# cocowy1/Cost-Volume-Aggregation-in-Stereo-Matching-Revisited

Measured on AMD Instinct MI355X. Metric: cost-volumes/sec (fwd+bwd) at 544x960 D=192, higher is better.
Workload: dtype f32

## Files before the change

### cost-volume-aggregation-in-stereo-matching-revisited_amd/csrc/abi.hip

```cpp
#include "dca_common.h"

extern "C" int dca_abi_version(void) { return DCA_ABI_VERSION; }

extern "C" int dca_tile_walk(long tiles, int grid, int wg, int* walk) {
  DCA_REQUIRE(walk && tiles >= 0 && tiles < DCA_TILES_END && grid > 0 && wg >= 0 && wg < grid);
  const DcaTileWalk w = dca_tile_walk_of(tiles, (unsigned)grid, (unsigned)wg);
  walk[0] = w.begin; walk[1] = w.end; walk[2] = w.step;
  return 0;
}
```

### cost-volume-aggregation-in-stereo-matching-revisited_amd/csrc/conv3d_wgrad_s2_f16x2.hip

```cpp
#include "dca_frag.h"
#include "dca_tiles.h"
#include <type_traits>

namespace {

constexpr int NT = 2;
constexpr int TH = 4, TW = 16;
constexpr int NROW = TH;
constexpr int FD = 3, FH = 2 * TH + 1, NFROW = FD * FH;
constexpr int FV = 2 * TW + 1;
constexpr int VB = 64;
constexpr int X_TERM = NFROW * FV * VB;
constexpr int Y_BLK = NROW * TW * VB;
constexpr int Y_TERM = 2 * Y_BLK;
constexpr int X_OFF = 0, Y_OFF = NT * X_TERM;
constexpr int LDS_BYTES = Y_OFF + NT * Y_TERM;
constexpr int NXQ = NFROW * 8 * 4;
constexpr int KXQ = (NXQ + 511) / 512;
constexpr int NXE = NFROW * 4;
constexpr int NYQ = 2 * NROW * 4 * 4;
static_assert(NXQ - 512 + NYQ <= 512, "coarse items fit behind the second round of fine items");

struct WS2Args {
  const float* x;
  const float* dy;
  float* part;
  int N, Cx, Cy, D, H, W;
  int Do, Ho, Wo;
  int nTD, nTH, nTW, nCxT, nCyP;
  const int* xexps;
  const int* yexps;
};

__global__ __launch_bounds__(512) void wgrad3s2_f16x2_kernel(WS2Args a) {
  extern __shared__ __attribute__((aligned(16))) char smem[];
  const int tid = threadIdx.x, lane = tid & 63, wv = tid >> 6, l31 = lane & 31, half = lane >> 5;
  const int blk = wv >> 2, wq = wv & 3;
  const int ct = blockIdx.y, cyp = ct / a.nCxT, cx0 = (ct % a.nCxT) * 32, cy0 = cyp * 64;
  const bool blk_on = cy0 + 32 * blk < a.Cy;

  const DcaTileWalk walk = dca_my_tile_walk((long)a.N * a.nTD * a.nTH * a.nTW);
  const int t_begin = walk.begin, t_end = walk.end, t_step = walk.step;

  f32x16 acc[7];
#pragma unroll
  for (int j = 0; j < 7; ++j)
#pragma unroll
    for (int r = 0; r < 16; ++r) acc[j][r] = 0.f;

  const int cstride = a.D * a.H * a.W, ystride = a.Do * a.Ho * a.Wo;
  const long xsample = (long)a.Cx * cstride, ysample = (long)a.Cy * ystride;

  const int q4 = (lane & 15) >> 2, chb = (16 * ((lane >> 4) & 1) + 4 * (lane & 3)) * 2;
  const int lane_off_x = (2 * (8 * half + q4)) * VB + chb;
  const int lane_off_y = (8 * half + q4) * VB + chb;

  float4 rq[KXQ][8];
  float re[8];
  int* ex_lds = (int*)(smem + LDS_BYTES);
  if (tid < 32) ex_lds[tid] = (cx0 + tid < a.Cx) ? dca_coherent_loadi(a.xexps + cx0 + tid) : 0;
  else if (tid < 96) ex_lds[tid] = (cy0 + tid - 32 < a.Cy) ? dca_coherent_loadi(a.yexps + cy0 + tid - 32) : 0;
  __syncthreads();
  const int yu = tid - (NXQ - 512);
  auto decode = [&](int tile, int& n, int& d0, int& h0, int& w0) __attribute__((always_inline)) {
    dca_tile_decode<1, TH, TW>(tile, a.nTD, a.nTH, a.nTW, n, d0, h0, w0);
  };
  auto load_tile = [&](int n, int d0, int h0, int w0, int part = -1) __attribute__((always_inline)) {
    const __amdgpu_buffer_rsrc_t xr = dca_rsrc(a.x + (long)n * xsample, xsample * 4);
    const __amdgpu_buffer_rsrc_t yr = dca_rsrc(a.dy + (long)n * ysample, ysample * 4);
#pragma unroll
    for (int k = 0; k < KXQ; ++k) {
      if ((part == 0 && k >= 1) || (part == 1 && k < 1)) continue;
      const int it = tid + 512 * k, cg = it & 3, quad = (it >> 2) & 7, frow = it >> 5;
      const int d = 2 * d0 - 1 + frow / FH, h = 2 * h0 - 1 + frow % FH, w = 2 * w0 + 4 * quad, c0 = cx0 + cg * 8;
      const int ok = (int)(it < NXQ) & (int)((unsigned)d < (unsigned)a.D) & (int)((unsigned)h < (unsigned)a.H) & (int)(w + 3 < a.W);
      const int off = (c0 * cstride + (d * a.H + h) * a.W + w) * 4;
      if (512 * k + (tid & ~63) < NXQ) {
#pragma unroll
        for (int j = 0; j < 8; ++j) rq[k][j] = dca_bload4(xr, off + j * cstride * 4, ok & (int)(c0 + j < a.Cx));
      }
    }
    if (part == 0) return;
    if ((tid & ~63) < NXE + 63) {
      const int cg = tid & 3, frow = tid >> 2, c0 = cx0 + cg * 8;
      const int d = 2 * d0 - 1 + frow / FH, h = 2 * h0 - 1 + frow % FH, w = 2 * w0 - 1;
      const int ok = (int)(tid < NXE) & (int)((unsigned)d < (unsigned)a.D) & (int)((unsigned)h < (unsigned)a.H) &
                     (int)((unsigned)w < (unsigned)a.W);
      const int off = (c0 * cstride + (d * a.H + h) * a.W + w) * 4;
#pragma unroll
      for (int j = 0; j < 8; ++j) re[j] = dca_bload1(xr, off + j * cstride * 4, ok & (int)(c0 + j < a.Cx));
    }
    if ((unsigned)yu < (unsigned)NYQ) {
      const int cg = yu & 3, quad = (yu >> 2) & 3, row = (yu >> 4) & 3, by = yu >> 6;
      const int h = h0 + row, w = w0 + 4 * quad, c0 = cy0 + 32 * by + cg * 8;
      const int ok = (int)(h < a.Ho) & (int)(w + 3 < a.Wo);
      const int off = (c0 * ystride + (d0 * a.Ho + h) * a.Wo + w) * 4;
#pragma unroll
      for (int j = 0; j < 8; ++j) rq[1][j] = dca_bload4(yr, off + j * ystride * 4, ok & (int)(c0 + j < a.Cy));
    }
  };
  auto split_word = [&](const float (&v)[8], const int* exp8, char* dst, int term_stride) __attribute__((always_inline)) {
    const int4 e0 = *(const int4*)exp8, e1 = *(const int4*)(exp8 + 4);
    const int ex[8] = {e0.x, e0.y, e0.z, e0.w, e1.x, e1.y, e1.z, e1.w};
    f16x8 hv, lv;
#pragma unroll
    for (int j = 0; j < 8; ++j) {
      _Float16 h, l;
      x2_split(v[j], ex[j], h, l);
      hv[j] = h; lv[j] = l;
    }
    *(f16x8*)dst = hv;
    *(f16x8*)(dst + term_stride) = lv;
  };
  auto quad_words = [&](const float4 (&q)[8], const int* ex, char* dst, int term_stride) __attribute__((always_inline)) {
    const float* q0 = (const float*)&q[0];
#pragma unroll
    for (int vv = 0; vv < 4; ++vv) {
      const float v[8] = {q0[vv], q0[4 + vv], q0[8 + vv], q0[12 + vv], q0[16 + vv], q0[20 + vv], q0[24 + vv], q0[28 + vv]};
      split_word(v, ex, dst + vv * VB, term_stride);
    }
  };
  auto store_tile = [&]() __attribute__((always_inline)) {
#pragma unroll
    for (int k = 0; k < KXQ; ++k) {
      const int it = tid + 512 * k, cg = it & 3, quad = (it >> 2) & 7, frow = it >> 5;
      if (it < NXQ) quad_words(rq[k], ex_lds + cg * 8, smem + X_OFF + (frow * FV + 1 + 4 * quad) * VB + cg * 16, X_TERM);
    }
    if (tid < NXE) {
      const int cg = tid & 3, frow = tid >> 2;
      const float v[8] = {re[0], re[1], re[2], re[3], re[4], re[5], re[6], re[7]};
      split_word(v, ex_lds + cg * 8, smem + X_OFF + (frow * FV) * VB + cg * 16, X_TERM);
    }
    if ((unsigned)yu < (unsigned)NYQ) {
      const int cg = yu & 3, quad = (yu >> 2) & 3, row = (yu >> 4) & 3, by = yu >> 6;
      quad_words(rq[1], ex_lds + 32 + 32 * by + cg * 8, smem + Y_OFF + by * Y_BLK + (row * TW + 4 * quad) * VB + cg * 16, Y_TERM);
    }
  };

  auto mfma_tile = [&](auto WQC, bool more, int next_tile) __attribute__((always_inline)) {
    constexpr int WQ = decltype(WQC)::value;
    constexpr int TAP0 = 7 * WQ, TAP1 = (TAP0 + 7 < 27) ? TAP0 + 7 : 27, NTAP = TAP1 - TAP0;
#pragma unroll 1
    for (int i = 0; i < NROW; ++i) {
      if ((i == 1 || i == 2) && more) {
        int nn, nd0, nh0, nw0;
        decode(next_tile, nn, nd0, nh0, nw0);
        load_tile(nn, nd0, nh0, nw0, i - 1);
      }
      if (blk_on) {
        const char* yb = smem + Y_OFF + blk * Y_BLK + (i * TW) * VB + lane_off_y;
        const char* xb = smem + X_OFF + ((2 * i) * FV) * VB + lane_off_x;
        f16x8 ay[NT];
#pragma unroll
        for (int term = 0; term < NT; ++term) ay[term] = tr_frag(yb + term * Y_TERM, 4 * VB);
        f16x8 bx[2][NT];
        auto load_b = [&](int tap, int slot) __attribute__((always_inline)) {
          const int kd = tap / 9, kh = (tap / 3) % 3, kw = tap % 3;
#pragma unroll
          for (int term = 0; term < NT; ++term)
            bx[slot][term] = tr_frag(xb + term * X_TERM + ((kd * FH + kh) * FV + kw) * VB, 8 * VB);
        };
        load_b(TAP0, 0);
#pragma unroll
        for (int j = 0; j < NTAP; ++j) {
          const int cur = j & 1;
          if (j + 1 < NTAP) load_b(TAP0 + j + 1, cur ^ 1);
          acc[j] = __builtin_amdgcn_mfma_f32_32x32x16_f16(ay[0], bx[cur][1], acc[j], 0, 0, 0);
          acc[j] = __builtin_amdgcn_mfma_f32_32x32x16_f16(ay[1], bx[cur][0], acc[j], 0, 0, 0);
          acc[j] = __builtin_amdgcn_mfma_f32_32x32x16_f16(ay[0], bx[cur][0], acc[j], 0, 0, 0);
          if (j + 1 < NTAP) {
            __builtin_amdgcn_sched_group_barrier(0x100, 2, 0);
            __builtin_amdgcn_sched_group_barrier(0x008, 1, 0);
            __builtin_amdgcn_sched_group_barrier(0x100, 2, 0);
            __builtin_amdgcn_sched_group_barrier(0x008, 2, 0);
          }
          __builtin_amdgcn_sched_barrier(0);
        }
      }
    }
  };

  if (t_begin < t_end) {
    int n, d0, h0, w0;
    decode(t_begin, n, d0, h0, w0);
    load_tile(n, d0, h0, w0);
    store_tile();
    __syncthreads();
#pragma unroll 1
    for (int tile = t_begin; tile < t_end; tile += t_step) {
      const bool more = tile + t_step < t_end;
      switch (wq) {
        case 0: mfma_tile(std::integral_constant<int, 0>{}, more, tile + t_step); break;
        case 1: mfma_tile(std::integral_constant<int, 1>{}, more, tile + t_step); break;
        case 2: mfma_tile(std::integral_constant<int, 2>{}, more, tile + t_step); break;
        default: mfma_tile(std::integral_constant<int, 3>{}, more, tile + t_step); break;
      }
      __syncthreads();
      if (more) store_tile();
      __syncthreads();
    }
  }

  if (blk_on) {
    const int xe_l = ex_lds[l31];
    int ninv[16];
#pragma unroll
    for (int r = 0; r < 16; ++r) ninv[r] = -(ex_lds[32 + 32 * blk + (r & 3) + 8 * (r >> 2) + 4 * half] + xe_l);
    const int nCT32 = a.nCxT * ((a.Cy + 31) / 32), ct32 = (2 * cyp + blk) * a.nCxT + (ct % a.nCxT);
    float* slab = a.part + ((long)blockIdx.x * nCT32 + ct32) * 27 * 1024;
#pragma unroll
    for (int j = 0; j < 7; ++j) {
      const int tap = 7 * wq + j;
      if (tap < 27) {
#pragma unroll
        for (int r = 0; r < 16; ++r) {
          const int co = (r & 3) + 8 * (r >> 2) + 4 * half;
          slab[tap * 1024 + co * 32 + l31] = ldexpf(acc[j][r], ninv[r]);
        }
      }
    }
  }
}

struct WS2Geom {
  int Do, Ho, Wo, nCxT, nCyP, nWG, nCT, nblk;
  DcaTileGrid t;
  long part_floats;
};
WS2Geom ws2_geometry(int N, int Cx, int Cy, int D, int H, int W) {
  WS2Geom g;
  g.Do = (D + 1) / 2; g.Ho = (H + 1) / 2; g.Wo = (W + 1) / 2;
  g.t = dca_tile_grid<1, TH, TW>(N, g.Do, g.Ho, g.Wo);
  g.nCxT = cdiv(Cx, 32); g.nCyP = cdiv(Cy, 64);
  g.nWG = g.nCxT * g.nCyP;
  g.nCT = g.nCxT * cdiv(Cy, 32);
  g.nblk = dca_persistent_grid(g.t.tiles, g.nWG);
  g.part_floats = (long)g.nblk * g.nCT * 27 * 1024;
  return g;
}

}

extern "C" long dca_conv3d_wgrad_s2_x2_workspace(int N, int Cx, int Cy, int D, int H, int W) {
  if (N <= 0 || Cx <= 0 || Cy <= 0 || D <= 0 || H <= 0 || W <= 0) return 0;
  return ws2_geometry(N, Cx, Cy, D, H, W).part_floats;
}

extern "C" int dca_conv3d_wgrad_s2_x2(const float* f, const int* f_exps, const float* c, const int* c_exps,
                                      float* part, float* dw, int N, int Cx, int Cy, int D, int H, int W, long s_cy,
                                      long s_cx, hipStream_t stream) {
  DCA_REQUIRE(f && c && part && dw && f_exps && c_exps && N > 0 && Cx > 0 && Cy > 0 && D > 0 && H > 0 && W > 0);
  WS2Args a;
  a.x = f; a.dy = c; a.part = part; a.xexps = f_exps; a.yexps = c_exps;
  a.N = N; a.Cx = Cx; a.Cy = Cy; a.D = D; a.H = H; a.W = W;
  const WS2Geom g = ws2_geometry(N, Cx, Cy, D, H, W);
  a.Do = g.Do; a.Ho = g.Ho; a.Wo = g.Wo;
  DCA_REQUIRE(W % 4 == 0 && a.Wo % 4 == 0 && ((((uintptr_t)f | (uintptr_t)c) & 15) == 0));
  DCA_REQUIRE((long)Cx * D * H * W * 4 < 0x7ffffff0L && (long)Cy * a.Do * a.Ho * a.Wo * 4 < 0x7ffffff0L);
  a.nTD = g.t.nTD; a.nTH = g.t.nTH; a.nTW = g.t.nTW; a.nCxT = g.nCxT; a.nCyP = g.nCyP;
  DCA_REQUIRE(g.t.fits() && g.nWG <= 65535);
  const int lds = LDS_BYTES + 96 * 4;
  hipError_t e = hipFuncSetAttribute((const void*)wgrad3s2_f16x2_kernel, hipFuncAttributeMaxDynamicSharedMemorySize, lds);
  if (e != hipSuccess) return (int)e;
  hipLaunchKernelGGL(wgrad3s2_f16x2_kernel, dim3(g.nblk, g.nWG), dim3(512), lds, stream, a);
  int st = dca_launch_status();
  if (st) return st;
  return dca_internal_wgrad_reduce(part, dw, g.nblk, g.nCxT, g.nCT, 27, Cy, Cx, s_cy, s_cx, stream);
}
```

### cost-volume-aggregation-in-stereo-matching-revisited_amd/csrc/dca_tiles.h

```cpp
#pragma once
#include <hip/hip_runtime.h>

struct DcaTileWalk {
  int begin, end, step;
};

__host__ __device__ __forceinline__ DcaTileWalk dca_tile_walk_of(long T, unsigned grid, unsigned wg) {
  const int nx = grid >= 8 ? 8 : 1, xcd = wg % nx;
  const int cnt = (grid - xcd + nx - 1) / nx;
  DcaTileWalk w;
  w.begin = (int)(T * xcd / nx) + wg / nx; w.end = (int)(T * (xcd + 1) / nx); w.step = cnt;
  return w;
}
__device__ __forceinline__ DcaTileWalk dca_my_tile_walk(long T) { return dca_tile_walk_of(T, gridDim.x, blockIdx.x); }

template <int TD, int TH, int TW>
__host__ __device__ __forceinline__ void dca_tile_decode(int tile, int nTD, int nTH, int nTW, int& n, int& d0, int& h0, int& w0) {
  const int tw = tile % nTW; tile /= nTW;
  const int th = tile % nTH; tile /= nTH;
  const int td = tile % nTD;
  n = tile / nTD;
  d0 = td * TD; h0 = th * TH; w0 = tw * TW;
}

struct DcaTileStep {
  int tile, chunk, n, d0, h0, w0;
};
template <int TD, int TH, int TW>
__host__ __device__ __forceinline__ void dca_tile_advance(DcaTileStep& c, int nchunk, const DcaTileWalk& walk, int nTD, int nTH,
                                                          int nTW) {
  if (c.chunk + 1 < nchunk) { ++c.chunk; return; }
  c.chunk = 0;
  c.tile += walk.step;
  if (c.tile < walk.end) dca_tile_decode<TD, TH, TW>(c.tile, nTD, nTH, nTW, c.n, c.d0, c.h0, c.w0);
}

constexpr long DCA_TILES_END = 0x7fffffffL;
struct DcaTileGrid {
  int nTD, nTH, nTW;
  long tiles;
  bool fits() const { return tiles < DCA_TILES_END; }
};
template <int TD, int TH, int TW>
static inline DcaTileGrid dca_tile_grid(int N, int D, int H, int W) {
  DcaTileGrid t;
  t.nTD = (D + TD - 1) / TD; t.nTH = (H + TH - 1) / TH; t.nTW = (W + TW - 1) / TW;
  t.tiles = (long)N * t.nTD * t.nTH * t.nTW;
  return t;
}
```

### include/dca_hip.h

```cpp
#ifndef DCA_HIP_H
#define DCA_HIP_H

#include <hip/hip_runtime_api.h>

#ifdef __cplusplus
extern "C" {
#endif

#define DCA_ABI_VERSION 21
int dca_abi_version(void);

#define DCA_BF16 1
#define DCA_FP16 2

int dca_gwc_volume_fwd(const float* ref, const float* tgt, float* vol, int B, int C, int H, int W, int maxdisp,
                       int num_groups, hipStream_t stream);
int dca_gwc_volume_bwd(const float* gvol, const float* ref, const float* tgt, float* gref, float* gtgt, int B, int C,
                       int H, int W, int maxdisp, int num_groups, hipStream_t stream);
long dca_gwc_volume_bwd_rows(int B, int C, int H, int W, int maxdisp, int num_groups);
int dca_concat_volume_fwd(const float* ref, const float* tgt, float* vol, int B, int C, int H, int W, int maxdisp,
                          hipStream_t stream);
int dca_concat_volume_bwd(const float* gvol, float* gref, float* gtgt, int B, int C, int H, int W, int maxdisp,
                          hipStream_t stream);

int dca_cost_volume_fwd(const float* const* refs, const float* const* tgts, const int* seg_channels, int nseg,
                        const float* cref, const float* ctgt, int Cc, void* vol, int B, int H, int W, int maxdisp,
                        int num_groups, int dtype, unsigned* vmax, hipStream_t stream);

int dca_softargmin_fwd(const float* x, float* out, int B, int K, long HW, int mode, hipStream_t stream);
int dca_softargmin_bwd(const float* aux, const float* g, float* gx, int B, int K, long HW, int mode,
                       hipStream_t stream);

int dca_up_softargmin_fwd(const float* logits, float* disp, int B, int n, int hc, int wc, int scale, hipStream_t stream);
int dca_up_softargmin_bwd(const float* logits, const float* gdisp, float* g1, float* glogits, int B, int n, int hc,
                          int wc, int scale, hipStream_t stream);

int dca_conv3d_prep_weight(const float* w, float* wt, int A, int B, int Apad, int Bpad, int K, int src_ab, int flip,
                           int Btotal, int b_off, hipStream_t stream);
int dca_conv3d_forward(const float* x, const float* x2, const float* wt, float* y, const float* scale,
                       const float* shift, const float* res_pre, const float* res_post, float slope, int N, int Cin,
                       int C1, int Cout, int CinPad, int CoutTotal, int co_off, int Di, int Hi, int Wi, int Do, int Ho,
                       int Wo, int ksize, int stride, int transposed, hipStream_t stream);
long dca_conv3d_wgrad_workspace(int N, int Cx, int Cy, int Do, int Ho, int Wo, int ksize, int stride);
int dca_conv3d_wgrad(const float* x, const float* dy, float* part, float* dw, int N, int Cx, int Cy, int Di, int Hi,
                     int Wi, int Do, int Ho, int Wo, int ksize, int stride, long s_cy, long s_cx, hipStream_t stream);

long dca_conv1_bwd_fused_workspace(int N, long S, int two);
int dca_conv1_bwd_fused(const float* dz, const float* y, const float* stats, const float* dgb, float slope, int training,
                        const float* x, const float* x2, const float* w, float* part, float* dx, float* dx2, float* dw,
                        long s_cy, long s_cx, int N, int C1, int C2, int Cout, long S, hipStream_t stream);

long dca_conv1_x3_weight_bytes(int A);
int dca_conv1_x3_prep_weight(const float* w, void* wfrag, int A, int Bn, int src_ab, int Btotal, int b_off,
                             hipStream_t stream);
int dca_conv1_x3_forward(const float* x, const float* x2, const void* wfrag, float* y, const float* scale,
                         const float* shift, const float* res_pre, const float* res_post, float slope, int N, int C1,
                         int C2, int Cout, int CoutTotal, int co_off, long S, hipStream_t stream);

int dca_conv3d_prep_many(const void* table, int n, hipStream_t stream);

int dca_tile_walk(long tiles, int grid, int wg, int* walk);

long dca_conv3d_x3_weight_bytes(int Cin, int Cout);
int dca_conv3d_x3_prep_weight(const float* w, void* wx, int A, int B, int src_ab, int flip, hipStream_t stream);
int dca_conv3d_x3_forward(const float* x, const void* wx, float* y, const float* scale, const float* shift,
                          const float* res_pre, const float* res_post, float slope, int N, int Cin, int Cout, int D,
                          int H, int W, hipStream_t stream);

int dca_deconv3d_x3_forward(const float* x, const void* wx, float* y, const float* scale, const float* shift,
                            const float* res_pre, const float* res_post, float slope, int N, int Cin, int Cout, int Di,
                            int Hi, int Wi, hipStream_t stream);

long dca_conv3d_x3_stats_chunks(int N, int Cout, int D, int H, int W);
int dca_conv3d_x3_forward_stats(const float* x, const void* wx, float* y, double* stat_part, int N, int Cin, int Cout,
                                int D, int H, int W, hipStream_t stream);
long dca_conv1_x3_stats_chunks(int N, long S);
int dca_conv1_x3_forward_stats(const float* x, const float* x2, const void* wfrag, float* y, double* stat_part, int N,
                               int C1, int C2, int Cout, int CoutTotal, int co_off, long S, hipStream_t stream);
long dca_deconv3d_x3_stats_chunks(int N, int Di, int Hi, int Wi);
int dca_deconv3d_x3_forward_stats(const float* x, const void* wx, float* y, double* stat_part, int N, int Cin, int Cout,
                                  int Di, int Hi, int Wi, hipStream_t stream);
int dca_bn_finalize_centered(const double* part, int nchunk, const float* gamma, const float* beta, float* running_mean,
                             float* running_var, float momentum, float eps, float* stats, int* zexps,
                             const unsigned* rpre_slots, int rpre_n, const unsigned* rpost_slots, int rpost_n, int C,
                             hipStream_t stream);

long dca_conv3d_wgrad_x3_workspace(int N, int Cx, int Cy, int D, int H, int W);
int dca_conv3d_wgrad_x3(const float* x, const float* dy, float* part, float* dw, int N, int Cx, int Cy, int D, int H,
                        int W, long s_cy, long s_cx, hipStream_t stream);

#define DCA_AMAX_CSLOTS 1024
int dca_cmax_f32(const float* x, int N, int C, long S, unsigned* slots, hipStream_t stream);
int dca_cmax_exps(const unsigned* slots, int nslots, int C, int* exps, hipStream_t stream);
long dca_conv3d_x2_weight_bytes(int Cin, int Cout);
int dca_conv3d_x2_prep_weight(const float* w, void* wx, int A, int B, int src_ab, int flip, const unsigned* x_slots,
                              int nslots, int* xexps, hipStream_t stream);
int dca_conv3d_x2_forward(const void* x, int packed, const int* xexps, const void* wx, float* y, const float* scale,
                          const float* shift, const float* res_pre, const float* res_post, float slope, unsigned* y_cmax,
                          int N, int Cin, int Cout, int D, int H, int W, hipStream_t stream);
long dca_conv3d_x2_stats_chunks(int N, int Cout, int D, int H, int W);
int dca_conv3d_x2_forward_stats(const void* x, int packed, const int* xexps, const void* wx, float* y, double* stat_part,
                                int N, int Cin, int Cout, int D, int H, int W, hipStream_t stream);
long dca_conv3d_wgrad_s2_x2_workspace(int N, int Cx, int Cy, int D, int H, int W);
int dca_conv3d_wgrad_s2_x2(const float* f, const int* f_exps, const float* c, const int* c_exps, float* part,
                           float* dw, int N, int Cx, int Cy, int D, int H, int W, long s_cy, long s_cx, hipStream_t stream);
long dca_conv3d_s2x2_weight_bytes(int Cin, int Cout);
int dca_conv3d_s2x2_prep_weight(const float* w, void* wx, int A, int B, int src_ab, int flip, const unsigned* x_slots,
                                int nslots, int* xexps, hipStream_t stream);
long dca_conv3d_s2x2_out_slots(int N, int Cout, int Di, int Hi, int Wi);
int dca_conv3d_s2x2_forward(const float* x, const int* xexps, const void* wx, float* y, const float* scale, const float* shift,
                            float slope, const float* res_post, unsigned* y_cmax, int N, int Cin, int Cout, int Di, int Hi, int Wi,
                            hipStream_t stream);
long dca_conv3d_wgrad_x2_workspace(int N, int Cx, int Cy, int D, int H, int W);
int dca_conv3d_wgrad_x2(const void* x, int x_packed, const int* xexps, const void* dy, int dy_packed, const int* yexps,
                        float* part, float* dw, int N, int Cx, int Cy, int D, int H, int W, long s_cy, long s_cx,
                        hipStream_t stream);

int dca_conv3d_c1_gather(const float* T, float* y, int N, int D, int H, int W, hipStream_t stream);
int dca_conv3d_c1_wgrad(const float* x, const float* dy, float* part, float* dw, int N, int C, int D, int H, int W,
                        hipStream_t stream);
int dca_conv3d_c1_expand(const float* dy, float* G, int N, int D, int H, int W, hipStream_t stream);
int dca_conv3d_c1_bwd_data(const float* dy, const float* w, float* dx, int N, int C, int D, int H, int W,
                           hipStream_t stream);

int dca_bn_num_chunks(int C, long S);
int dca_bn_pack_chunks(int C, long S);
int dca_bn_stats(const float* x, double* part, int N, int C, long S, hipStream_t stream);
int dca_bn_finalize(const double* part, int nchunk, double count, const float* gamma, const float* beta,
                    float* running_mean, float* running_var, float momentum, float eps, int training, float* stats,
                    int* zexps, const unsigned* rpre_slots, int rpre_n, const unsigned* rpost_slots, int rpost_n, int C,
                    hipStream_t stream);
int dca_bn_apply(const float* y, const float* stats, const float* res_pre, const float* res_post, float* z, int N,
                 int C, long S, float slope, unsigned* zmax, unsigned* ymax, hipStream_t stream);
int dca_bn_apply_pack(const float* y, const float* stats, const int* zexps, void* zp, int N, int C, long S, float slope,
                      unsigned* ymax, const float* res_pre, const float* res_post, float* zf, unsigned* zmax,
                      hipStream_t stream);
int dca_bn_backward(const float* dz, const float* y, const float* res_pre, const float* stats, double* part,
                    float* dgb, float* dy, float* g_out, int N, int C, long S, float slope, int training,
                    unsigned* dmax, hipStream_t stream);
int dca_bn_backward_reduce(const float* dz, const float* y, const float* stats, double* part, float* dgb, int N, int C,
                           long S, float slope, int training, hipStream_t stream);
int dca_bn_backward_pack(const float* dz, const float* y, const float* stats, double* part, float* dgb, void* dyp,
                         int* dyexps, unsigned* gmax, const unsigned* ymax, int ymax_slots, int N, int C, long S,
                         float slope, int training, hipStream_t stream);
int dca_bn_skip_max(const float* y_r, const float* stats_r, int N, int C, long S, unsigned* slots, hipStream_t stream);
int dca_bn_apply_pack_skip(const float* y, const float* stats, const int* zexps, void* zp, int N, int C, long S, float slope,
                           unsigned* ymax, const float* y_r, const float* stats_r, const float* res_post, float* zf,
                           unsigned* zmax, hipStream_t stream);
int dca_bn_backward_skip(const float* dz, const float* y, const float* y_r, const float* stats, const float* stats_r,
                         double* part, double* part_r, float* dgb, float* dgb_r, float* dy, float* g_out, int N, int C,
                         long S, float slope, int training, unsigned* dmax, hipStream_t stream);

int dca_avgpool3d_fwd(const float* x, float* y, long NC, int Di, int Hi, int Wi, hipStream_t stream);
int dca_avgpool3d_bwd(const float* gy, float* gx, const float* res, const float* res2, long NC, int Di, int Hi, int Wi,
                     hipStream_t stream);

int dca_trilinear_fwd(const float* x, float* y, long NC, int Di, int Hi, int Wi, int scale, hipStream_t stream);
int dca_trilinear_bwd(const float* gy, float* gx, long NC, int Di, int Hi, int Wi, int scale, hipStream_t stream);

int dca_context_inject_fwd(const float* x, const float* preds, float* key, int* kstar, float* e, float* pm,
                           float* denom, float* part, int B, int C, int n, long HW, hipStream_t stream);
int dca_context_inject_bwd(const float* dkey, const float* x, const float* preds, const int* kstar, const float* e,
                           const float* pm, const float* denom, float* dx, float* dpreds, float* dw, float* T,
                           float* part, int B, int C, int n, long HW, hipStream_t stream);

int dca_disp_attention_fwd(const float* q, const float* k, const float* v, float* out, int B, int C, int n, long HW,
                           hipStream_t stream);
int dca_disp_attention_bwd(const float* q, const float* k, const float* v, const float* dout, float* dq, float* dk,
                           float* dv, int B, int C, int n, long HW, hipStream_t stream);

int dca_convex_up4_fwd(const float* mask_logits, const float* disp, float* up, int B, int h, int w, hipStream_t stream);
int dca_convex_up4_bwd(const float* mask_logits, const float* disp, const float* gup, float* glogits, float* gdisp,
                       float* wk, int B, int h, int w, hipStream_t stream);

long dca_focal_loss_workspace(int nlev, int B, long HW);
int dca_focal_loss_fwd(const float* const* ests, const float* weights, int nlev, const float* gt, double* work,
                       float* out, int B, int K, long HW, float focal_coefficient, hipStream_t stream);
int dca_focal_loss_bwd(const float* const* ests, float* const* gests, const float* weights, int nlev, const float* gt,
                       const double* work, const float* gloss, int B, int K, long HW, float focal_coefficient,
                       hipStream_t stream);

long dca_conv3d_lp_weight_bytes(int Cin, int Cout);
int dca_conv3d_lp_prep_weight(const float* w, void* wx, int A, int B, int src_ab, int flip, int dtype,
                              hipStream_t stream);
int dca_conv3d_lp_forward(const void* x, const void* wx, void* y, const float* scale, const float* shift,
                          const void* res_pre, const void* res_post, float slope, int N, int Cin, int Cout, int D, int H,
                          int W, int dtype, int in_f32, int out_f32, hipStream_t stream);

long dca_conv1_lp_weight_bytes(int C1, int C2);
int dca_conv1_lp_prep_weight(const float* w, void* wfrag, int Cout, int C1, int C2, int dtype, hipStream_t stream);
int dca_conv1_lp_forward(const void* x, const void* x2, const void* wfrag, void* y, const float* scale,
                         const float* shift, const void* res_pre, const void* res_post, float slope, int N, int C1,
                         int C2, int Cout, long S, int dtype, int out_f32, hipStream_t stream);

int dca_conv3d_forward_mixed(const void* x, const float* wt, void* y, const float* scale, const float* shift,
                             const void* res_pre, const void* res_post, float slope, int N, int Cin, int Cout, int CinPad,
                             int Di, int Hi, int Wi, int Do, int Ho, int Wo, int transposed, int dtype,
                             hipStream_t stream);
long dca_conv3d_s2_lp_weight_bytes(int Cin);
int dca_conv3d_s2_lp_prep_weight(const float* w, void* wx, int Cin, int Cout, int dtype, hipStream_t stream);
int dca_conv3d_s2_lp_forward(const void* x, const void* wx, float* y, const float* scale, const float* shift, float slope,
                             int N, int Cin, int Cout, int D, int H, int W, int dtype, hipStream_t stream);
int dca_deconv3d_lp_forward(const float* x, const void* wx, void* y, const float* scale, const float* shift,
                            const void* res_pre, const void* res_post, float slope, int N, int Cin, int Cout, int Di,
                            int Hi, int Wi, int dtype, hipStream_t stream);
int dca_avgpool3d_lp_fwd(const void* x, float* y, long NC, int Di, int Hi, int Wi, int dtype, hipStream_t stream);
int dca_trilinear_up2_lp_fwd(const float* x, void* y, long NC, int Di, int Hi, int Wi, int dtype, hipStream_t stream);

#define DCA_EVAL_REC 8
long dca_disp_metrics_workspace(int B, int H, int W);
int dca_disp_metrics(const float* pred, const float* gt, const unsigned char* mask, double* rec, void* workspace, int B,
                     int H, int W, int top_pad, int right_pad, float maxdisp, hipStream_t stream);
#define DCA_EVAL_MAX_CLASSES 64
int dca_region_confusion(const float* vol0, const float* vol1, const float* vol2, const float* gt, long long* cm,
                         int nvol, int B, int C, int hp, int wp, int H, int W, hipStream_t stream);
#define DCA_EVAL_BATCHES 0
#define DCA_EVAL_SUMS 1
#define DCA_EVAL_IMG_KEPT 11
#define DCA_EVAL_IMG_EPE 12
#define DCA_EVAL_IMG_D1 13
#define DCA_EVAL_IMG_THRES 14
#define DCA_EVAL_IMG_SEEN 17
#define DCA_EVAL_PIXELS 18
#define DCA_EVAL_STATE_HEAD 32
long dca_eval_state_len(int C);
int dca_eval_accumulate(const double* rec, const long long* cm, double* state, int B, int nvol, int C, int H, int W,
                        hipStream_t stream);

int dca_frame_hist(const unsigned char* left, const unsigned char* right, unsigned* hist, int H, int W, int C,
                   hipStream_t stream);
int dca_frame_lut(const unsigned* hist, long n_pixels, float* lut, double* stats, hipStream_t stream);
int dca_frame_apply(const unsigned char* left, const unsigned char* right, const float* lut, float* out_left,
                    float* out_right, int H, int W, int C, int Hc, int Wc, int src_y0, int dst_y0, int rows, int cols,
                    hipStream_t stream);
int dca_disp_export(const float* pred, float* out_f32, unsigned short* out_u16, int Hc, int Wc, int y0, int h, int w,
                    float scale, hipStream_t stream);

int dca_train_luma_sum(const unsigned char* left, const unsigned char* right, const unsigned char* bg, long long* S, int H,
                       int W, int C, hipStream_t stream);
int dca_train_tables(const long long* S, long n_pixels, const unsigned char* bg, float f_left, float f_right,
                     const float* norm, unsigned char* U, float* T, hipStream_t stream);
int dca_train_patch_colour(const unsigned char* right, const unsigned char* U, long long* sums, unsigned char* colour,
                           int H, int W, int C, int y1, int x1, int th, int tw, hipStream_t stream);
int dca_train_crop_norm(const unsigned char* left, const unsigned char* right, const float* T, const float* norm,
                        const unsigned char* colour, float* out_left, float* out_right, int H, int W, int C, int y1, int x1,
                        int th, int tw, int py0, int px0, int ph, int pw, hipStream_t stream);
int dca_train_disp_crop(const void* src, int src_u16, float* gt, unsigned char* mask, int H, int W, int y1, int x1, int th,
                        int tw, int flip_rows, float scale, int inf_to_zero, float maxdisp, hipStream_t stream);

#define DCA_CONF_DISP 0
#define DCA_CONF_DUNI 1
#define DCA_CONF_MASS 2
#define DCA_CONF_ENT 3
#define DCA_CONF_STD 4
#define DCA_CONF_PLANES 5
int dca_softargmin_stats(const float* logits, float* out, int B, int K, long HW, int radius, hipStream_t stream);
#define DCA_CONF_MAX_PLANES 8
int dca_convex_up4_planes(const float* mask_logits, const float* planes, const float* scales, float* up, int B, int P,
                          int h, int w, hipStream_t stream);
#define DCA_CONF_MAX_BINS 1024
#define DCA_CONF_ERR_SCALE 1048576
int dca_conf_histogram(const float* conf, const float* pred, const float* gt, long long* state, int B, long HW, int nbins,
                       float maxdisp, hipStream_t stream);

#define DCA_LR_MAX_W 8192
int dca_mirror_pair(const float* left, const float* right, float* out_left, float* out_right, int N, int H, int W,
                    hipStream_t stream);
int dca_lr_consistency(const float* dl, const float* drm, float* diff, float* valid, float* filled, float* disp_right,
                       int B, int H, int W, int cols, float tau, hipStream_t stream);

#define DCA_PC_TILE 1024
#define DCA_PC_RECORD_BYTES 16
int dca_disp_to_depth(const float* pred, const float* mask, float* out_f32, unsigned short* out_u16, int Hc, int Wc, int y0,
                      int rows, int cols, float fb, float doffs, float min_disp, float max_depth, float mask_min,
                      float scale, hipStream_t stream);
long dca_point_cloud_tiles(int rows, int cols);
int dca_point_cloud(const float* pred, const float* mask, const unsigned char* rgb, int C, int Hsrc, int Wsrc, void* vertices,
                    long cap, unsigned* tile_offsets, long long* count, int Hc, int Wc, int y0, int rows, int cols, int v0,
                    int stride, float f, float fb, float cx, float cy, float doffs, float min_disp, float max_depth,
                    float mask_min, hipStream_t stream);

#define DCA_SELFSUP_MAX_LEVELS 8
#define DCA_SELFSUP_TILE_W 64
#define DCA_SELFSUP_TILE_H 16
#define DCA_SELFSUP_SUMS 4
#define DCA_SELFSUP_OUT 5
int dca_selfsup_loss_fwd(const float* left, const float* right, const float* const* disps, const float* weights, int nlev,
                         const void* valid, int valid_u8, double* work, float* out, int B, int H, int W, float alpha,
                         float lam, float c1, float c2, float photo_scale, hipStream_t stream);
int dca_selfsup_loss_bwd(const float* left, const float* right, const float* const* disps, float* const* gdisps,
                         const float* weights, int nlev, const void* valid, int valid_u8, const float* out,
                         const float* gloss, int B, int H, int W, float alpha, float lam, float c1, float c2,
                         float photo_scale, hipStream_t stream);

#define DCA_RECT_FRAC_BITS 5
#define DCA_RECT_MAX_SRC 16384
int dca_rectify_pair(const unsigned char* left, const unsigned char* right, const int* maps, long map_plane,
                     unsigned char* out_left, unsigned char* out_right, int Hs, int Ws, int Hd, int Wd, int C,
                     hipStream_t stream);

#define DCA_ERRMAP_BINS 10
#define DCA_ERRMAP_RGB_0 0x313695
#define DCA_ERRMAP_RGB_1 0x4575B4
#define DCA_ERRMAP_RGB_2 0x74ADD1
#define DCA_ERRMAP_RGB_3 0xABD9E9
#define DCA_ERRMAP_RGB_4 0xE0F3F8
#define DCA_ERRMAP_RGB_5 0xFEE090
#define DCA_ERRMAP_RGB_6 0xFDAE61
#define DCA_ERRMAP_RGB_7 0xF46D43
#define DCA_ERRMAP_RGB_8 0xD73027
#define DCA_ERRMAP_RGB_9 0xA50026
#define DCA_ERRMAP_LEGEND_ROWS 10
#define DCA_ERRMAP_LEGEND_STEP 20
int dca_disp_error_image(const float* pred, const float* gt, float* out_f32, unsigned char* out_u8, int B, int H, int W,
                         int top_pad, int right_pad, float abs_thres, float rel_thres, int legend, hipStream_t stream);
long dca_disp_range_workspace(int B, int rows, int cols);
int dca_disp_range(const float* disp, const float* mask, float* range, void* workspace, int B, int Hc, int Wc, int y0,
                   int rows, int cols, float mask_min, hipStream_t stream);
#define DCA_CMAP_GRAY 0
#define DCA_CMAP_KITTI 1
#define DCA_KITTI_EDGE_0 0
#define DCA_KITTI_EDGE_1 114
#define DCA_KITTI_EDGE_2 299
#define DCA_KITTI_EDGE_3 413
#define DCA_KITTI_EDGE_4 587
#define DCA_KITTI_EDGE_5 701
#define DCA_KITTI_EDGE_6 886
#define DCA_KITTI_EDGE_7 1000
#define DCA_KITTI_CORNERS 0x76325410
int dca_disp_colorize(const float* disp, const float* mask, const float* range, unsigned char* out_u8, int Hc, int Wc, int y0,
                      int rows, int cols, float max_disp, float mask_min, int cmap, hipStream_t stream);

#define DCA_LIDAR_MAX_RADIUS 8
int dca_lidar_disparity(const float* points, long N, int S, long n, float m00, float m01, float m02, float m03, float m10,
                        float m11, float m12, float m13, float m20, float m21, float m22, float m23, int H, int W, float fb,
                        float doffs, float min_depth, float max_depth, float min_disp, float max_disp, int rx, int ry,
                        double rel, float* disp, float* depth, unsigned short* disp_u16, long long* count, unsigned* zbuf,
                        hipStream_t stream);

#define DCA_SPK_TILE_H 16
#define DCA_SPK_TILE_W 64
int dca_speckle_filter(const float* d, const float* mask, float* out_disp, float* out_valid, int* out_size, int* label,
                       int* count, int B, int Hc, int Wc, int y0, int rows, int cols, int max_size, float max_diff,
                       float mask_min, float fill, hipStream_t stream);
int dca_median_filter(const float* d, const float* mask, float* out, int B, int Hc, int Wc, int y0, int rows, int cols,
                      int ksize, float mask_min, hipStream_t stream);

#define DCA_HR_MAX_SCALE 4
#define DCA_HR_MAX_RADIUS 3
#define DCA_HR_RANGE_LEN 766
#define DCA_HR_THREADS 256
#define DCA_HR_TILE_H 16
#define DCA_HR_TILE_W 64
#define DCA_HR_RUN 4
int dca_area_downscale_u8(const unsigned char* left, const unsigned char* right, unsigned char* out, int H, int W, int C,
                          int s, hipStream_t stream);
int dca_area_downscale_f32(const float* in, float* out, int H, int W, int s, int inf_to_zero, int flip_rows,
                           hipStream_t stream);
int dca_guided_upsample(const float* disp_lo, const float* mask_lo, const unsigned char* guide_lo,
                        const unsigned char* guide_hi, const float* ws, const float* wr, float* out, float* valid, int Hc,
                        int Wc, int y0, int rows, int cols, int H, int W, int C, int s, int r, float mask_min,
                        hipStream_t stream);

#ifdef __cplusplus
}
#endif
#endif
```

Measured before the change: 43.94.

## Reuse overlapping depth planes via LDS ring buffer in stride-2 wgrad kernel

Each workgroup now walks a contiguous run of tiles with depth varying fastest, so consecutive tiles share one of the three input depth planes. The x staging area becomes a 3-plane ring buffer. Successor tiles load and split only the two new planes, and the MFMA loop indexes planes through the ring offset. This cuts global loads and f16 split work for x by about a third, but changes the tile-to-workgroup distribution from strided to contiguous runs, which may affect load balance and L2 locality.

Measured after the change: 44.30, median of 6. No clear change (+0.8%).

```diff
diff --git a/cost-volume-aggregation-in-stereo-matching-revisited_amd/csrc/abi.hip b/cost-volume-aggregation-in-stereo-matching-revisited_amd/csrc/abi.hip
--- a/cost-volume-aggregation-in-stereo-matching-revisited_amd/csrc/abi.hip
+++ b/cost-volume-aggregation-in-stereo-matching-revisited_amd/csrc/abi.hip
@@ -8,3 +8,17 @@
   walk[0] = w.begin; walk[1] = w.end; walk[2] = w.step;
   return 0;
 }
+
+extern "C" int dca_tile_run(long tiles, int grid, int wg, int* run) {
+  DCA_REQUIRE(run && tiles >= 0 && tiles < DCA_TILES_END && grid > 0 && wg >= 0 && wg < grid);
+  const DcaTileWalk w = dca_tile_run_of(tiles, (unsigned)grid, (unsigned)wg);
+  run[0] = w.begin; run[1] = w.end;
+  return 0;
+}
+
+extern "C" int dca_tile_run_decode(int tile, int nTD, int nTH, int nTW, int* ntdhw) {
+  DCA_REQUIRE(ntdhw && tile >= 0 && nTD > 0 && nTH > 0 && nTW > 0);
+  int d0;
+  dca_tile_decode_dfast<1, 1, 1>(tile, nTD, nTH, nTW, ntdhw[0], ntdhw[1], d0, ntdhw[2], ntdhw[3]);
+  return 0;
+}
diff --git a/cost-volume-aggregation-in-stereo-matching-revisited_amd/csrc/conv3d_wgrad_s2_f16x2.hip b/cost-volume-aggregation-in-stereo-matching-revisited_amd/csrc/conv3d_wgrad_s2_f16x2.hip
--- a/cost-volume-aggregation-in-stereo-matching-revisited_amd/csrc/conv3d_wgrad_s2_f16x2.hip
+++ b/cost-volume-aggregation-in-stereo-matching-revisited_amd/csrc/conv3d_wgrad_s2_f16x2.hip
@@ -10,7 +10,8 @@
 constexpr int FD = 3, FH = 2 * TH + 1, NFROW = FD * FH;
 constexpr int FV = 2 * TW + 1;
 constexpr int VB = 64;
-constexpr int X_TERM = NFROW * FV * VB;
+constexpr int X_PLANE = FH * FV * VB;
+constexpr int X_TERM = FD * X_PLANE;
 constexpr int Y_BLK = NROW * TW * VB;
 constexpr int Y_TERM = 2 * Y_BLK;
 constexpr int X_OFF = 0, Y_OFF = NT * X_TERM;
@@ -18,6 +19,7 @@
 constexpr int NXQ = NFROW * 8 * 4;
 constexpr int KXQ = (NXQ + 511) / 512;
 constexpr int NXE = NFROW * 4;
+constexpr int NXQ_S = 2 * FH * 8 * 4, NXE_S = 2 * FH * 4;
 constexpr int NYQ = 2 * NROW * 4 * 4;
 static_assert(NXQ - 512 + NYQ <= 512, "coarse items fit behind the second round of fine items");
 
@@ -39,8 +41,8 @@
   const int ct = blockIdx.y, cyp = ct / a.nCxT, cx0 = (ct % a.nCxT) * 32, cy0 = cyp * 64;
   const bool blk_on = cy0 + 32 * blk < a.Cy;
 
-  const DcaTileWalk walk = dca_my_tile_walk((long)a.N * a.nTD * a.nTH * a.nTW);
-  const int t_begin = walk.begin, t_end = walk.end, t_step = walk.step;
+  const DcaTileWalk run = dca_my_tile_run((long)a.N * a.nTD * a.nTH * a.nTW);
+  const int t_begin = run.begin, t_end = run.end;
 
   f32x16 acc[7];
 #pragma unroll
@@ -62,29 +64,37 @@
   else if (tid < 96) ex_lds[tid] = (cy0 + tid - 32 < a.Cy) ? dca_coherent_loadi(a.yexps + cy0 + tid - 32) : 0;
   __syncthreads();
   const int yu = tid - (NXQ - 512);
+  auto fresh_tid = [&]() __attribute__((always_inline)) {
+    int t = tid;
+    asm volatile("" : "+v"(t));
+    return t;
+  };
   auto decode = [&](int tile, int& n, int& d0, int& h0, int& w0) __attribute__((always_inline)) {
-    dca_tile_decode<1, TH, TW>(tile, a.nTD, a.nTH, a.nTW, n, d0, h0, w0);
-  };
-  auto load_tile = [&](int n, int d0, int h0, int w0, int part = -1) __attribute__((always_inline)) {
+    int td;
+    dca_tile_decode_dfast<1, TH, TW>(tile, a.nTD, a.nTH, a.nTW, n, td, d0, h0, w0);
+  };
+  auto load_tile = [&](int n, int d0, int h0, int w0, bool succ, int part = -1) __attribute__((always_inline)) {
+    const int row0 = succ ? FH : 0, nxq = succ ? NXQ_S : NXQ, nxe = succ ? NXE_S : NXE;
+    const int tid = fresh_tid();
     const __amdgpu_buffer_rsrc_t xr = dca_rsrc(a.x + (long)n * xsample, xsample * 4);
     const __amdgpu_buffer_rsrc_t yr = dca_rsrc(a.dy + (long)n * ysample, ysample * 4);
 #pragma unroll
     for (int k = 0; k < KXQ; ++k) {
       if ((part == 0 && k >= 1) || (part == 1 && k < 1)) continue;
-      const int it = tid + 512 * k, cg = it & 3, quad = (it >> 2) & 7, frow = it >> 5;
+      const int it = tid + 512 * k, cg = it & 3, quad = (it >> 2) & 7, frow = row0 + (it >> 5);
       const int d = 2 * d0 - 1 + frow / FH, h = 2 * h0 - 1 + frow % FH, w = 2 * w0 + 4 * quad, c0 = cx0 + cg * 8;
-      const int ok = (int)(it < NXQ) & (int)((unsigned)d < (unsigned)a.D) & (int)((unsigned)h < (unsigned)a.H) & (int)(w + 3 < a.W);
+      const int ok = (int)(it < nxq) & (int)((unsigned)d < (unsigned)a.D) & (int)((unsigned)h < (unsigned)a.H) & (int)(w + 3 < a.W);
       const int off = (c0 * cstride + (d * a.H + h) * a.W + w) * 4;
-      if (512 * k + (tid & ~63) < NXQ) {
+      if (512 * k + (tid & ~63) < nxq) {
 #pragma unroll
         for (int j = 0; j < 8; ++j) rq[k][j] = dca_bload4(xr, off + j * cstride * 4, ok & (int)(c0 + j < a.Cx));
       }
     }
     if (part == 0) return;
-    if ((tid & ~63) < NXE + 63) {
-      const int cg = tid & 3, frow = tid >> 2, c0 = cx0 + cg * 8;
+    if ((tid & ~63) < nxe) {
+      const int cg = tid & 3, frow = row0 + (tid >> 2), c0 = cx0 + cg * 8;
       const int d = 2 * d0 - 1 + frow / FH, h = 2 * h0 - 1 + frow % FH, w = 2 * w0 - 1;
-      const int ok = (int)(tid < NXE) & (int)((unsigned)d < (unsigned)a.D) & (int)((unsigned)h < (unsigned)a.H) &
+      const int ok = (int)(tid < nxe) & (int)((unsigned)d < (unsigned)a.D) & (int)((unsigned)h < (unsigned)a.H) &
                      (int)((unsigned)w < (unsigned)a.W);
       const int off = (c0 * cstride + (d * a.H + h) * a.W + w) * 4;
 #pragma unroll
@@ -120,16 +130,23 @@
       split_word(v, ex, dst + vv * VB, term_stride);
     }
   };
-  auto store_tile = [&]() __attribute__((always_inline)) {
+  auto ring_row = [&](int frow, int sbase) __attribute__((always_inline)) {
+    const int kd = frow / FH, s = sbase + kd;
+    return (s >= FD ? s - FD : s) * X_PLANE + (frow - kd * FH) * (FV * VB);
+  };
+  auto store_tile = [&](bool succ, int sbase) __attribute__((always_inline)) {
+    const int row0 = succ ? FH : 0, nxq = succ ? NXQ_S : NXQ, nxe = succ ? NXE_S : NXE;
+    const int tid = fresh_tid();
 #pragma unroll
     for (int k = 0; k < KXQ; ++k) {
-      const int it = tid + 512 * k, cg = it & 3, quad = (it >> 2) & 7, frow = it >> 5;
-      if (it < NXQ) quad_words(rq[k], ex_lds + cg * 8, smem + X_OFF + (frow * FV + 1 + 4 * quad) * VB + cg * 16, X_TERM);
-    }
-    if (tid < NXE) {
-      const int cg = tid & 3, frow = tid >> 2;
+      const int it = tid + 512 * k, cg = it & 3, quad = (it >> 2) & 7, frow = row0 + (it >> 5);
+      if (it < nxq)
+        quad_words(rq[k], ex_lds + cg * 8, smem + X_OFF + ring_row(frow, sbase) + (1 + 4 * quad) * VB + cg * 16, X_TERM);
+    }
+    if (tid < nxe) {
+      const int cg = tid & 3, frow = row0 + (tid >> 2);
       const float v[8] = {re[0], re[1], re[2], re[3], re[4], re[5], re[6], re[7]};
-      split_word(v, ex_lds + cg * 8, smem + X_OFF + (frow * FV) * VB + cg * 16, X_TERM);
+      split_word(v, ex_lds + cg * 8, smem + X_OFF + ring_row(frow, sbase) + cg * 16, X_TERM);
     }
     if ((unsigned)yu < (unsigned)NYQ) {
       const int cg = yu & 3, quad = (yu >> 2) & 3, row = (yu >> 4) & 3, by = yu >> 6;
@@ -137,19 +154,24 @@
     }
   };
 
-  auto mfma_tile = [&](auto WQC, bool more, int next_tile) __attribute__((always_inline)) {
+  auto mfma_tile = [&](auto WQC, int sbase, bool more, int next_tile, bool next_succ) __attribute__((always_inline)) {
     constexpr int WQ = decltype(WQC)::value;
     constexpr int TAP0 = 7 * WQ, TAP1 = (TAP0 + 7 < 27) ? TAP0 + 7 : 27, NTAP = TAP1 - TAP0;
+    constexpr int KD_LO = TAP0 / 9, KD_HI = (TAP1 - 1) / 9;
+    static_assert(KD_HI - KD_LO <= 1, "a tap group spans at most two planes");
+    const int s_lo = sbase + KD_LO, s_hi = sbase + KD_HI;
+    const int p_lo = (s_lo >= FD ? s_lo - FD : s_lo) * X_PLANE, p_hi = (s_hi >= FD ? s_hi - FD : s_hi) * X_PLANE;
 #pragma unroll 1
     for (int i = 0; i < NROW; ++i) {
-      if ((i == 1 || i == 2) && more) {
+      if ((i == 0 || i == 1) && more) {
         int nn, nd0, nh0, nw0;
         decode(next_tile, nn, nd0, nh0, nw0);
-        load_tile(nn, nd0, nh0, nw0, i - 1);
+        load_tile(nn, nd0, nh0, nw0, next_succ, i);
       }
       if (blk_on) {
         const char* yb = smem + Y_OFF + blk * Y_BLK + (i * TW) * VB + lane_off_y;
-        const char* xb = smem + X_OFF + ((2 * i) * FV) * VB + lane_off_x;
+        const char* xb_lo = smem + X_OFF + p_lo + ((2 * i) * FV) * VB + lane_off_x;
+        const char* xb_hi = smem + X_OFF + p_hi + ((2 * i) * FV) * VB + lane_off_x;
         f16x8 ay[NT];
 #pragma unroll
         for (int term = 0; term < NT; ++term) ay[term] = tr_frag(yb + term * Y_TERM, 4 * VB);
@@ -158,7 +180,7 @@
           const int kd = tap / 9, kh = (tap / 3) % 3, kw = tap % 3;
 #pragma unroll
           for (int term = 0; term < NT; ++term)
-            bx[slot][term] = tr_frag(xb + term * X_TERM + ((kd * FH + kh) * FV + kw) * VB, 8 * VB);
+            bx[slot][term] = tr_frag((kd == KD_LO ? xb_lo : xb_hi) + term * X_TERM + (kh * FV + kw) * VB, 8 * VB);
         };
         load_b(TAP0, 0);
 #pragma unroll
@@ -183,20 +205,24 @@
   if (t_begin < t_end) {
     int n, d0, h0, w0;
     decode(t_begin, n, d0, h0, w0);
-    load_tile(n, d0, h0, w0);
-    store_tile();
+    int td = d0, sbase = (2 * td + 2) % FD;
+    load_tile(n, d0, h0, w0, false);
+    store_tile(false, sbase);
     __syncthreads();
 #pragma unroll 1
-    for (int tile = t_begin; tile < t_end; tile += t_step) {
-      const bool more = tile + t_step < t_end;
+    for (int tile = t_begin; tile < t_end; ++tile) {
+      const bool more = tile + 1 < t_end;
+      const bool succ = td + 1 < a.nTD;
       switch (wq) {
-        case 0: mfma_tile(std::integral_constant<int, 0>{}, more, tile + t_step); break;
-        case 1: mfma_tile(std::integral_constant<int, 1>{}, more, tile + t_step); break;
-        case 2: mfma_tile(std::integral_constant<int, 2>{}, more, tile + t_step); break;
-        default: mfma_tile(std::integral_constant<int, 3>{}, more, tile + t_step); break;
-      }
+        case 0: mfma_tile(std::integral_constant<int, 0>{}, sbase, more, tile + 1, succ); break;
+        case 1: mfma_tile(std::integral_constant<int, 1>{}, sbase, more, tile + 1, succ); break;
+        case 2: mfma_tile(std::integral_constant<int, 2>{}, sbase, more, tile + 1, succ); break;
+        default: mfma_tile(std::integral_constant<int, 3>{}, sbase, more, tile + 1, succ); break;
+      }
+      td = succ ? td + 1 : 0;
+      sbase = (2 * td + 2) % FD;
       __syncthreads();
-      if (more) store_tile();
+      if (more) store_tile(succ, sbase);
       __syncthreads();
     }
   }
diff --git a/cost-volume-aggregation-in-stereo-matching-revisited_amd/csrc/dca_tiles.h b/cost-volume-aggregation-in-stereo-matching-revisited_amd/csrc/dca_tiles.h
--- a/cost-volume-aggregation-in-stereo-matching-revisited_amd/csrc/dca_tiles.h
+++ b/cost-volume-aggregation-in-stereo-matching-revisited_amd/csrc/dca_tiles.h
@@ -20,6 +20,26 @@
   const int th = tile % nTH; tile /= nTH;
   const int td = tile % nTD;
   n = tile / nTD;
+  d0 = td * TD; h0 = th * TH; w0 = tw * TW;
+}
+
+__host__ __device__ __forceinline__ DcaTileWalk dca_tile_run_of(long T, unsigned grid, unsigned wg) {
+  const int nx = grid >= 8 ? 8 : 1, xcd = wg % nx;
+  const int cnt = (grid - xcd + nx - 1) / nx;
+  const long b = T * xcd / nx, len = T * (xcd + 1) / nx - b, j = wg / nx;
+  DcaTileWalk w;
+  w.begin = (int)(b + len * j / cnt); w.end = (int)(b + len * (j + 1) / cnt); w.step = 1;
+  return w;
+}
+__device__ __forceinline__ DcaTileWalk dca_my_tile_run(long T) { return dca_tile_run_of(T, gridDim.x, blockIdx.x); }
+
+template <int TD, int TH, int TW>
+__host__ __device__ __forceinline__ void dca_tile_decode_dfast(int tile, int nTD, int nTH, int nTW, int& n, int& td, int& d0, int& h0,
+                                                               int& w0) {
+  td = tile % nTD; tile /= nTD;
+  const int tw = tile % nTW; tile /= nTW;
+  const int th = tile % nTH;
+  n = tile / nTH;
   d0 = td * TD; h0 = th * TH; w0 = tw * TW;
 }
 
diff --git a/include/dca_hip.h b/include/dca_hip.h
--- a/include/dca_hip.h
+++ b/include/dca_hip.h
@@ -60,6 +60,8 @@
 int dca_conv3d_prep_many(const void* table, int n, hipStream_t stream);
 
 int dca_tile_walk(long tiles, int grid, int wg, int* walk);
+int dca_tile_run(long tiles, int grid, int wg, int* run);
+int dca_tile_run_decode(int tile, int nTD, int nTH, int nTW, int* ntdhw);
 
 long dca_conv3d_x3_weight_bytes(int Cin, int Cout);
 int dca_conv3d_x3_prep_weight(const float* w, void* wx, int A, int B, int src_ab, int flip, hipStream_t stream);
```
